# Fedomn/sqlrs

Hardware: AMD Instinct MI355X
Metric: Mrows/sec for filter->hash-join->group-by pipeline; achieved HBM GB/s vs peak (higher is better)
Workload: dtype int64 keys / f64 sum; 1 GPU; C5 filter(val>0.5) -> hash-join(fact x dim on int64 key) -> group-by(key) COUNT,SUM(f64); fact_rows=1000000000, dim_rows=10000000, groups=10000000, parallelism=single GPU

## Files before the change

sqlrs_amd/csrc/agg_partition.hip:

```cpp
#include <algorithm>
#include <cstdlib>
#include <cstring>

#include "agg_partition.hpp"
#include "device_utils.hpp"
#include "radix_part.hpp"

namespace sq {

#ifndef PART_WG_N
#define PART_WG_N 512
#endif
constexpr int PART_WG = PART_WG_N;
#ifndef DENSE_WG_N
#define DENSE_WG_N 1024
#endif
constexpr int DENSE_WG = DENSE_WG_N;
#ifndef HOT_MIN_PEERS_N
#define HOT_MIN_PEERS_N 8
#endif
constexpr int HOT_MIN_PEERS = HOT_MIN_PEERS_N;
constexpr uint64_t LDS_EMPTY = ~0ull;

__device__ __forceinline__ uint32_t bucket_of(uint64_t h, uint32_t P) {
// ... 1351 lines not shown
  out->may_dup = false;
  uint32_t nsplit = 0, nchunk_tables = 0;
  for (uint32_t bkt = 0; bkt < P; bkt++) {
    uint32_t lo = hb[bkt], hi = pr.bucket_end(bkt);
    if (dense && lo == hi) continue;
    if (hi - lo <= split_above) {
      work.insert(work.end(), {bkt, lo, hi, 0xffffffffu});
    } else if (dense) {
      chunk_lo.push_back(nchunk_tables);
      const uint32_t pieces = (uint32_t)ceil_div((int64_t)(hi - lo), (int64_t)chunk);
      for (uint32_t q = 0; q < pieces; q++) {
        const uint32_t c0 = lo + (uint32_t)((uint64_t)(hi - lo) * q / pieces), c1 = lo + (uint32_t)((uint64_t)(hi - lo) * (q + 1) / pieces);
        work.insert(work.end(), {bkt, c0, c1, nchunk_tables++});
      }
      split_bucket.push_back(bkt);
      nsplit++;
    } else {
      for (uint32_t c0 = lo; c0 < hi; c0 += chunk) work.insert(work.end(), {bkt, c0, std::min(hi, c0 + chunk), nsplit});
      split_bucket.push_back(bkt);
      nsplit++;
    }
  }
  chunk_lo.push_back(nchunk_tables);
  if (nsplit) {
    std::vector<uint32_t> ord(work.size() / 4), sorted(work.size());
    for (uint32_t i = 0; i < ord.size(); i++) ord[i] = i;
    std::stable_sort(ord.begin(), ord.end(), [&](uint32_t a, uint32_t b) {
      return work[4 * a + 2] - work[4 * a + 1] > work[4 * b + 2] - work[4 * b + 1];
    });
    for (size_t i = 0; i < ord.size(); i++) std::memcpy(&sorted[4 * i], &work[4 * ord[i]], 16);
    work.swap(sorted);
  }
  const uint32_t nwork = (uint32_t)(work.size() / 4);
  BufP dwork = ctx->alloc(4 * work.size() + 16);
  SQ_HIP(hipMemcpyAsync(dwork->p, work.data(), 4 * work.size(), hipMemcpyHostToDevice, ctx->stream));
  const uint32_t nslots_h = dense ? cap : cap + 2;
  SplitTables stb;
  BufP stb_key, stb_first, stb_acc, dsplit;
  BufP dchunk_lo;
  if (nsplit && dense) {
    const int64_t total = (int64_t)nchunk_tables * nslots_h;
    stb_first = ctx->alloc(4 * (size_t)total);
    stb_acc = ctx->alloc(8 * (size_t)total * (size_t)std::max(spec.n_acc, 1));
    stb.first = stb_first->as<unsigned int>();
    stb.acc = stb_acc->as<unsigned long long>();
    stb.nsplit = nchunk_tables;
    dsplit = ctx->alloc(4 * (size_t)nsplit);
    dchunk_lo = ctx->alloc(4 * ((size_t)nsplit + 1));
    SQ_HIP(hipMemcpyAsync(dsplit->p, split_bucket.data(), 4 * (size_t)nsplit, hipMemcpyHostToDevice, ctx->stream));
    SQ_HIP(hipMemcpyAsync(dchunk_lo->p, chunk_lo.data(), 4 * ((size_t)nsplit + 1), hipMemcpyHostToDevice, ctx->stream));
  } else if (nsplit) {
    const int64_t total = (int64_t)nsplit * nslots_h;
    stb_key = ctx->alloc(8 * (size_t)total);
    stb_first = ctx->alloc(4 * (size_t)total);
    stb_acc = ctx->alloc(8 * (size_t)total * (size_t)std::max(spec.n_acc, 1));
    stb.key = stb_key->as<unsigned long long>();
    stb.first = stb_first->as<unsigned int>();
    stb.acc = stb_acc->as<unsigned long long>();
    stb.nsplit = nsplit;
    split_init_kernel<<<dim3((unsigned)ceil_div(total, 256)), dim3(256), 0, ctx->stream>>>(stb, total, spec.n_acc, prm);
    SQ_HIP(hipGetLastError());
  }
  out->gkey = ctx->alloc(8 * (size_t)gcap);
  out->gfirst = ctx->alloc(4 * (size_t)gcap);
  out->gvalid = in.key_validity ? ctx->alloc((size_t)gcap) : nullptr;
  out->gacc = ctx->alloc(8 * (size_t)gcap * (size_t)std::max(spec.n_acc, 1));
  out->gcap = gcap;
  if (!out->ov_rows) out->ov_rows = ctx->alloc(4 * (size_t)std::max<int64_t>(n, 1));
  ctx->agg_route[pr.pack.kbits ? Ctx::AR_PACKED : Ctx::AR_UNPACKED]++;
  ctx->agg_route[Ctx::AR_FLAGS] += pf != nullptr;
  ctx->agg_route[Ctx::AR_REC] += pr.rec != nullptr;
  ctx->agg_route[Ctx::AR_IN_PLACE] += in_place;
  ctx->agg_route[Ctx::AR_JOIN] += join_mode;
  ctx->agg_route[Ctx::AR_JOIN_MULT] += prm.partner_mult != nullptr;
  ctx->agg_route[Ctx::AR_SPLIT] += nsplit > 0;
  {
    ProfScope ps(ctx, "lds_agg");
#define SQ_LA(NV, FL, JN, NA, C0, C1, PK)                                                                        \
  do {                                                                                                         \
    auto kfn = lds_agg_kernel<NV, FL, JN, NA, C0, C1, PK>;                                                      \
    constexpr bool can_rec = NV == 1 && PK && !FL;                                                             \
    if (can_rec && pr.rec) kfn = lds_agg_kernel<NV, FL, JN, NA, C0, C1, PK, can_rec>;                          \
    else if (pr.rec) fail(SQLRS_ERR_INTERNAL, "record-form partition in a column-form bucket pass");           \
    allow_big_lds(ctx, kfn);                                                                                   \
    kfn<<<dim3(nwork), dim3(PART_WG), lds, ctx->stream>>>(                                                     \
        prm, pr.rec ? pr.rec->as<uint64_t>() : pk->as<uint64_t>(), pi ? pi->as<uint32_t>() : nullptr, pv0 ? pv0->as<uint64_t>() : nullptr,       \
        pv1 ? pv1->as<uint64_t>() : nullptr, pf ? pf->as<uint8_t>() : nullptr, dwork->as<uint32_t>(), P, n,    \
        ctr->as<unsigned long long>(), out->gkey->as<uint64_t>(), out->gfirst->as<uint32_t>(),                 \
        out->gvalid ? out->gvalid->as<uint8_t>() : nullptr, out->gacc->as<uint64_t>(), gcap,                   \
        ctr->as<unsigned long long>() + 1, out->ov_rows->as<uint32_t>(),                                       \
        bp ? bp->key->as<uint64_t>() : nullptr, (bp && bp->flags) ? bp->flags->as<uint8_t>() : nullptr,        \
        bp ? bp->bstart->as<uint32_t>() : nullptr, pr.pack, stb);                                              \
    ctx->agg_route[NA < 0 ? Ctx::AR_PROBE_GENERIC : Ctx::AR_PROBE_SPEC]++;                                     \
    launched = true;                                                                                           \
  } while (0)
#define SQ_LA_J(NV, FL, NA, C0, C1)                                                                            \
  do {                                                                                                         \
    if (pr.pack.kbits) {                                                                                       \
      if (join_mode) SQ_LA(NV, FL, true, NA, C0, C1, true);                                                    \
      else SQ_LA(NV, FL, false, NA, C0, C1, true);                                                             \
    } else {                                                                                                   \
      if (join_mode) SQ_LA(NV, FL, true, NA, C0, C1, false);                                                   \
      else SQ_LA(NV, FL, false, NA, C0, C1, false);                                                            \
    }                                                                                                          \
  } while (0)
    const int nvu = pv1 ? 2 : ((pv0 || pr.rec) ? 1 : 0);
    bool launched = false;
    if (dense && pr.slim.on) {
// ... 131 lines not shown
```

sqlrs_amd/csrc/common.hpp:

```cpp
#pragma once

#include <hip/hip_runtime.h>

#include <cstdint>
#include <cstdlib>
#include <cstring>
#include <map>
#include <set>
#include <memory>
#include <string>
#include <vector>

#include "sqlrs_hip.h"

namespace sq {

inline bool hooks_enabled() {
  static const bool on = [] {
    const char *e = std::getenv("SQLRS_HOOKS");
    return e && e[0] == '1';
  }();
  return on;
}
inline const char *hook(const char *name) { return hooks_enabled() ? std::getenv(name) : nullptr; }
// ... 64 lines not shown
  Buf &operator=(const Buf &) = delete;
  template <class T> T *as() const { return (T *)p; }
};
using BufP = std::shared_ptr<Buf>;
inline BufP buf_view(const BufP &parent, const void *p, size_t bytes) {
  BufP v = std::make_shared<Buf>(parent->ctx, const_cast<void *>(p), bytes);
  v->owned = false;
  v->parent = parent;
  return v;
}

struct ProfEntry {
  const char *name;
  double total_ms = 0;
  int64_t launches = 0;
};
struct ProfPending {
  int entry;
  hipEvent_t a, b;
};

struct Ctx {
  int device = 0;
  hipStream_t stream = nullptr;
  std::string last_error;
  std::shared_ptr<Pool> pool_ref = std::make_shared<Pool>();
  Pool &pool = *pool_ref;
  int num_cus = 256;
  bool prof_on = false;
  std::vector<ProfEntry> prof;
  std::vector<ProfPending> prof_pending;
  std::vector<hipEvent_t> event_pool;
  hipEvent_t order_event = nullptr;
  void *pinned = nullptr;
  size_t pinned_bytes = 0;

  BufP alloc(size_t bytes);
  BufP alloc_zero(size_t bytes);
  BufP zero_block;
  size_t zero_used = 0;
  std::set<const void *> big_lds_set;
  std::map<const void *, int> occ_cache;
  int64_t lb_timeouts = 0;
  int64_t order_lb_fallbacks = 0;
  int lb_backoff = 0;
  int64_t async_conj_batches = 0;
  int64_t async_fast_batches = 0;
  enum AggRoute {
    AR_DENSE, AR_SLIM_RUNS, AR_SLIM_BLK, AR_PROBE_SPEC, AR_PROBE_GENERIC,
    AR_INTERPRETED,
    AR_PACKED, AR_UNPACKED,
    AR_FLAGS,
    AR_REC,
    AR_IN_PLACE,
    AR_JOIN,
    AR_JOIN_MULT,
    AR_SPLIT,
    AR_OVERFLOW_ROWS,
    AR_MERGE_GROUPS,
    AR_PENDING,
    AR_WIDE_PARTS,
    AR_COUNT_
  };
  int64_t agg_route[AR_COUNT_] = {};
  std::shared_ptr<void> small_ring;
  void sync() { SQ_HIP(hipStreamSynchronize(stream)); }
  const void *fetch(const void *dptr, size_t bytes);
  template <class T> T fetch_value(const T *dptr) { return *(const T *)fetch(dptr, sizeof(T)); }
  void *pinned_early = nullptr;
  hipEvent_t early_event = nullptr;
  bool fetch_early(const void *dptr, size_t bytes);
  const void *fetch_early_wait();
  int prof_entry(const char *name);
  void prof_resolve();
};

template <class K> inline void allow_big_lds(Ctx *ctx, K kfn, int bytes = 150 * 1024) {
  const void *f = (const void *)kfn;
  if (ctx->big_lds_set.count(f)) return;
  SQ_HIP(hipFuncSetAttribute(f, hipFuncAttributeMaxDynamicSharedMemorySize, bytes));
  ctx->big_lds_set.insert(f);
}

struct ProfScope {
  Ctx *ctx;
  int entry = -1;
  hipEvent_t a = nullptr, b = nullptr;
  ProfScope(Ctx *c, const char *name);
  ~ProfScope();
};

struct DCol {
  int32_t dtype = SQLRS_NULLTYPE;
  int64_t length = 0;
  int64_t null_count = 0;
  int stride = 1;
  const void *values = nullptr;
  const uint64_t *validity = nullptr;
  const int32_t *offsets = nullptr;
  int64_t data_bytes = 0;
  uint64_t scalar_bits = 0;
  bool scalar_null = false;
  BufP own_values, own_validity, own_offsets;
  bool has_nulls() const { return validity != nullptr && null_count != 0; }
  template <class T> const T *v() const { return (const T *)values; }
};

struct DBatch {
  int64_t rows = 0;
  std::vector<DCol> cols;
};

struct InBatch {
  Ctx *ctx;
  const sqlrs_batch_t *abi;
  std::vector<DCol> cache;
  std::vector<uint8_t> loaded;
  bool host_upload = false;
  const DBatch *shared = nullptr;
  InBatch(Ctx *c, const sqlrs_batch_t *b);
  ~InBatch();
  InBatch(const InBatch &) = delete;
// ... 65 lines not shown
```

sqlrs_amd/csrc/ctx.hip:

```cpp
#include <cstdlib>

#include <array>
#include <atomic>
#include <mutex>
#include <unordered_set>

#include "common.hpp"
#include "host_stage.hpp"
#include "prims.hpp"
#include "small_async.hpp"

extern "C" void sqlrs_batch_release(sqlrs_batch_t *batch);
namespace sq {

static size_t pool_size_class(size_t bytes) {
  if (bytes < 512) return 512;
  if (bytes <= (1u << 20)) {
    size_t s = 512;
    while (s < bytes) s <<= 1;
    return s;
  }
  return round_up(bytes, (size_t)2 << 20);
}

// ... 153 lines not shown
const void *Ctx::fetch(const void *dptr, size_t bytes) {
  if (bytes > pinned_bytes) fail(SQLRS_ERR_INTERNAL, "fetch too large");
  SQ_HIP(hipMemcpyAsync(pinned, dptr, bytes, hipMemcpyDeviceToHost, stream));
  sync();
  return pinned;
}
bool Ctx::fetch_early(const void *dptr, size_t bytes) {
  if (bytes > pinned_bytes) return false;
  if (!pinned_early && hipHostMalloc(&pinned_early, pinned_bytes, hipHostMallocDefault) != hipSuccess) {
    pinned_early = nullptr;
    return false;
  }
  if (!early_event && hipEventCreateWithFlags(&early_event, hipEventDisableTiming) != hipSuccess) {
    early_event = nullptr;
    return false;
  }
  SQ_HIP(hipMemcpyAsync(pinned_early, dptr, bytes, hipMemcpyDeviceToHost, stream));
  SQ_HIP(hipEventRecord(early_event, stream));
  return true;
}
const void *Ctx::fetch_early_wait() {
  SQ_HIP(hipEventSynchronize(early_event));
  return pinned_early;
}
int Ctx::prof_entry(const char *name) {
  for (size_t i = 0; i < prof.size(); i++)
    if (prof[i].name == name || std::strcmp(prof[i].name, name) == 0) return (int)i;
  prof.push_back(ProfEntry{name});
  return (int)prof.size() - 1;
}
void Ctx::prof_resolve() {
  if (prof_pending.empty()) return;
  sync();
  for (auto &p : prof_pending) {
    float ms = 0;
    if (hipEventElapsedTime(&ms, p.a, p.b) == hipSuccess) {
      prof[p.entry].total_ms += ms;
      prof[p.entry].launches++;
    }
    event_pool.push_back(p.a);
    event_pool.push_back(p.b);
  }
  prof_pending.clear();
}

ProfScope::ProfScope(Ctx *c, const char *name) : ctx(c) {
  if (!c->prof_on) return;
  entry = c->prof_entry(name);
  auto get = [&]() {
    if (!c->event_pool.empty()) {
      hipEvent_t e = c->event_pool.back();
      c->event_pool.pop_back();
      return e;
    }
    hipEvent_t e;
    SQ_HIP(hipEventCreate(&e));
    return e;
  };
  a = get();
  b = get();
  (void)hipEventRecord(a, c->stream);
}
ProfScope::~ProfScope() {
  if (entry < 0) return;
  (void)hipEventRecord(b, ctx->stream);
  ctx->prof_pending.push_back(ProfPending{entry, a, b});
  if (ctx->prof_pending.size() > 4096) {
    try {
      ctx->prof_resolve();
    } catch (...) {
    }
  }
}

Expr expr_from_abi(const sqlrs_expr_t *e) {
  Expr x;
  if (!e || e->num_nodes <= 0 || !e->nodes) fail(SQLRS_ERR_INTERNAL, "empty expression");
  x.nodes.assign(e->nodes, e->nodes + e->num_nodes);
  x.strings.resize(x.nodes.size());
  for (size_t i = 0; i < x.nodes.size(); i++) {
    if (x.nodes[i].s) x.strings[i] = x.nodes[i].s;
    x.nodes[i].s = nullptr;
  }
  return x;
}

static void copy_in(Ctx *ctx, void *dst, const void *src, size_t bytes, int mem) {
  if (!bytes) return;
  SQ_HIP(hipMemcpyAsync(dst, src, bytes,
                        mem == SQLRS_MEM_HOST ? hipMemcpyHostToDevice : hipMemcpyDeviceToDevice,
                        ctx->stream));
}

DCol upload_column(Ctx *ctx, const sqlrs_column_t &c, bool force_copy) {
  DCol d;
  d.dtype = c.dtype;
  d.length = c.length;
  d.null_count = c.validity ? c.null_count : 0;
// ... 501 lines not shown
  int n = 0;
  if (hipGetDeviceCount(&n) != hipSuccess || n <= 0 || device_id < 0 || device_id >= n)
    return SQLRS_ERR_DEVICE;
  hipDeviceProp_t prop;
  if (hipGetDeviceProperties(&prop, device_id) != hipSuccess) return SQLRS_ERR_DEVICE;
  if (std::string(prop.gcnArchName).rfind("gfx950", 0) != 0) return SQLRS_ERR_DEVICE;
  if (hipSetDevice(device_id) != hipSuccess) return SQLRS_ERR_DEVICE;
  auto *c = new sqlrs_ctx();
  c->device = device_id;
  c->pool.device = device_id;
  c->num_cus = prop.multiProcessorCount;
  if (hipStreamCreateWithFlags(&c->stream, hipStreamNonBlocking) != hipSuccess ||
      hipHostMalloc(&c->pinned, 65536, hipHostMallocDefault) != hipSuccess) {
    delete c;
    return SQLRS_ERR_DEVICE;
  }
  c->pinned_bytes = 65536;
  if (const char *e = std::getenv("SQLRS_POOL_RESERVE_GB")) {
    const size_t bytes = (size_t)(std::atof(e) * (double)(1ull << 30));
    void *p = nullptr;
    if (bytes && hipMalloc(&p, bytes) == hipSuccess) {
      c->pool.arena = (uint8_t *)p;
      c->pool.arena_bytes = bytes;
    }
  }
  *out = c;
  return SQLRS_OK;
}

void sqlrs_ctx_destroy(sqlrs_ctx_t *ctx) {
  if (!ctx) return;
  (void)hipSetDevice(ctx->device);
  (void)hipStreamSynchronize(ctx->stream);
  for (auto &p : ctx->prof_pending) {
    (void)hipEventDestroy(p.a);
    (void)hipEventDestroy(p.b);
  }
  for (auto e : ctx->event_pool) (void)hipEventDestroy(e);
  if (ctx->order_event) (void)hipEventDestroy(ctx->order_event);
  ctx->zero_block.reset();
  ctx->pool.trim();
  if (ctx->pool.arena && ctx->pool.live_bytes == 0) {
    ctx->pool.free_blocks.clear();
    (void)hipFree(ctx->pool.arena);
    ctx->pool.arena = nullptr;
  }
  ctx->pool.closed = true;
  if (ctx->pinned) (void)hipHostFree(ctx->pinned);
  if (ctx->pinned_early) (void)hipHostFree(ctx->pinned_early);
  if (ctx->early_event) (void)hipEventDestroy(ctx->early_event);
  (void)hipStreamDestroy(ctx->stream);
  delete ctx;
}

const char *sqlrs_last_error(const sqlrs_ctx_t *ctx) { return ctx ? ctx->last_error.c_str() : ""; }

int sqlrs_ctx_synchronize(sqlrs_ctx_t *ctx) {
  return guard(ctx, [&] {
    ctx->sync();
    sa_drain(ctx);
  });
}
void *sqlrs_ctx_stream(sqlrs_ctx_t *ctx) { return (void *)ctx->stream; }

static int order_streams(sqlrs_ctx_t *ctx, hipStream_t first, hipStream_t then) {
  return guard(ctx, [&] {
    SQ_HIP(hipSetDevice(ctx->device));
    if (!ctx->order_event) SQ_HIP(hipEventCreateWithFlags(&ctx->order_event, hipEventDisableTiming));
    SQ_HIP(hipEventRecord(ctx->order_event, first));
    SQ_HIP(hipStreamWaitEvent(then, ctx->order_event, 0));
  });
}
int sqlrs_ctx_wait_stream(sqlrs_ctx_t *ctx, void *producer_stream) {
  return order_streams(ctx, (hipStream_t)producer_stream, ctx->stream);
}
int sqlrs_ctx_release_to_stream(sqlrs_ctx_t *ctx, void *consumer_stream) {
  return order_streams(ctx, ctx->stream, (hipStream_t)consumer_stream);
}
int64_t sqlrs_ctx_pool_bytes(const sqlrs_ctx_t *ctx) {
  return (int64_t)(ctx->pool.live_bytes + ctx->pool.cached_bytes);
}
void sqlrs_ctx_pool_trim(sqlrs_ctx_t *ctx) {
  (void)hipStreamSynchronize(ctx->stream);
// ... 381 lines not shown
```

sqlrs_amd/csrc/gather.hip:

```cpp
#include "common.hpp"
#include "device_utils.hpp"
#include "prims.hpp"

namespace sq {

template <class T, class I>
__global__ __launch_bounds__(BLOCK) void gather_kernel(const T *__restrict__ src,
                                                       const uint64_t *__restrict__ src_validity,
                                                       const I *__restrict__ idx,
                                                       const uint64_t *__restrict__ idx_validity,
                                                       int64_t n, T *__restrict__ out,
                                                       uint64_t *__restrict__ out_validity) {
  int64_t i = blockIdx.x * (int64_t)blockDim.x + threadIdx.x;
  bool in_range = i < n;
  bool valid = in_range;
  I s = 0;
  if (in_range) {
    if (idx_validity) valid = (idx_validity[i >> 6] >> (i & 63)) & 1;
    if (valid) {
      s = idx[i];
      if (src_validity) valid = (src_validity[s >> 6] >> (s & 63)) & 1;
    }
    out[i] = valid ? src[s] : T(0);
  }
// ... 180 lines not shown
  if (K > 2) {
    u64x2 b;
    b.x = c2[i];
    b.y = K > 3 ? c3[i] : 0ull;
    *(u64x2 *)(rows + (size_t)W * i + 2) = b;
  }
}
template <int K>
__global__ __launch_bounds__(BLOCK) void gather_rows_kernel(const uint64_t *__restrict__ rows, const uint32_t *__restrict__ idx,
                                                            int64_t n, uint64_t *__restrict__ o0, uint64_t *__restrict__ o1,
                                                            uint64_t *__restrict__ o2, uint64_t *__restrict__ o3) {
  constexpr int W = K <= 2 ? 2 : 4, U = 4;
  const int64_t base = blockIdx.x * (int64_t)(BLOCK * U) + threadIdx.x;
  uint32_t s[U];
#pragma unroll
  for (int u = 0; u < U; u++) s[u] = __builtin_nontemporal_load(idx + min(base + u * BLOCK, n - 1));
  u64x2 a[U], b[U];
#pragma unroll
  for (int u = 0; u < U; u++) {
    a[u] = *(const u64x2 *)(rows + (size_t)W * s[u]);
    if (K > 2) b[u] = *(const u64x2 *)(rows + (size_t)W * s[u] + 2);
  }
#pragma unroll
  for (int u = 0; u < U; u++) {
    const int64_t i = base + u * BLOCK;
    if (i >= n) continue;
    o0[i] = a[u].x;
    o1[i] = a[u].y;
    if (K > 2) o2[i] = b[u].x;
    if (K > 3) o3[i] = b[u].y;
  }
}

bool gather_columns_packed(Ctx *ctx, std::vector<DCol> &cols, int64_t src_rows, const uint32_t *idx, int64_t n) {
  const int k = (int)cols.size();
  if (k < 2 || k > 4 || n < (1 << 18)) return false;
  for (const DCol &c : cols)
    if (width_of(c.dtype) != 8 || c.stride == 0 || (c.validity && c.null_count != 0) || c.length != src_rows) return false;
  const int w = k <= 2 ? 2 : 4;
  BufP rows = ctx->alloc(8 * (size_t)w * (size_t)src_rows);
  const uint64_t *p[4] = {nullptr, nullptr, nullptr, nullptr};
  for (int i = 0; i < k; i++) p[i] = cols[(size_t)i].v<uint64_t>();
  dim3 b(BLOCK), gp((unsigned)ceil_div(src_rows, BLOCK)), gg((unsigned)ceil_div(n, BLOCK * 4));
  std::vector<DCol> outs((size_t)k);
  uint64_t *o[4] = {nullptr, nullptr, nullptr, nullptr};
  for (int i = 0; i < k; i++) {
    DCol &d = outs[(size_t)i];
    d.dtype = cols[(size_t)i].dtype;
    d.length = n;
    d.null_count = 0;
    d.own_values = ctx->alloc(8 * (size_t)n + 16);
    d.values = d.own_values->p;
    o[i] = d.own_values->as<uint64_t>();
  }
  uint64_t *r = rows->as<uint64_t>();
  switch (k) {
  case 2:
    pack_rows_kernel<2><<<gp, b, 0, ctx->stream>>>(p[0], p[1], p[2], p[3], src_rows, r);
    gather_rows_kernel<2><<<gg, b, 0, ctx->stream>>>(r, idx, n, o[0], o[1], o[2], o[3]);
    break;
  case 3:
    pack_rows_kernel<3><<<gp, b, 0, ctx->stream>>>(p[0], p[1], p[2], p[3], src_rows, r);
    gather_rows_kernel<3><<<gg, b, 0, ctx->stream>>>(r, idx, n, o[0], o[1], o[2], o[3]);
    break;
  default:
    pack_rows_kernel<4><<<gp, b, 0, ctx->stream>>>(p[0], p[1], p[2], p[3], src_rows, r);
    gather_rows_kernel<4><<<gg, b, 0, ctx->stream>>>(r, idx, n, o[0], o[1], o[2], o[3]);
  }
  SQ_HIP(hipGetLastError());
  cols = std::move(outs);
  return true;
}

__global__ void count_clear_kernel(const uint64_t *__restrict__ bits, int64_t rows, int64_t nwords,
                                   unsigned long long *out) {
  int64_t i = blockIdx.x * (int64_t)blockDim.x + threadIdx.x;
  uint64_t c = 0;
  for (int64_t w = i; w < nwords; w += (int64_t)gridDim.x * blockDim.x) {
    uint64_t v = ~bits[w];
    int64_t rem = rows - w * 64;
    if (rem < 64) v &= (1ull << rem) - 1;
    c += (uint64_t)__popcll(v);
  }
  c = wave_sum_u64(c);
  if (lane_id() == 0 && c) atomicAdd(out, (unsigned long long)c);
}
int64_t count_clear_bits(Ctx *ctx, const uint64_t *bits, int64_t rows) {
  if (!bits || rows == 0) return 0;
  BufP out = ctx->alloc_zero(8);
  int64_t nwords = ceil_div(rows, 64);
  unsigned blocks = (unsigned)std::min<int64_t>(ceil_div(nwords, 256), 2048);
  count_clear_kernel<<<dim3(blocks), dim3(256), 0, ctx->stream>>>(
      bits, rows, nwords, out->as<unsigned long long>());
  SQ_HIP(hipGetLastError());
  return (int64_t)ctx->fetch_value(out->as<uint64_t>());
}

__global__ void append_bits_kernel(const uint64_t *__restrict__ src, int64_t n, int64_t dst_off,
                                   unsigned long long *__restrict__ dst, int all_ones) {
  int64_t i = blockIdx.x * (int64_t)blockDim.x + threadIdx.x;
  int64_t nw = (n + 63) >> 6;
  if (i >= nw) return;
  uint64_t v = all_ones ? ~0ull : src[i];
// ... 200 lines not shown
```

sqlrs_amd/csrc/hashagg_op.hip:

```cpp
#include <cstdlib>

#include "agg_partition.hpp"
#include "agg_state.hpp"
#include "common.hpp"
#include "device_utils.hpp"
#include "host_stage.hpp"
#include "prims.hpp"

using namespace sq;

namespace {

struct AggSpec {
  int func = 0, distinct = 0;
  int32_t return_dtype = 0;
  Expr arg;
  GrowBuf acc, nn;
  bool track_nn = false;
  int32_t acc_dtype = 0;
  int argcol = -1;
  struct StrBatch {
    DCol col;
    BufP gid;
    int64_t n;
// ... 253 lines not shown
    int col = pg.col_of_agg[i];
    int cc = pg.cnt_of_col[(size_t)col];
    if (s.func == SQLRS_AGG_COUNT) {
      s.nn.ensure(ctx, G, 0);
      agg_update_count(ctx, s.nn, rg, nullptr, (const int64_t *)cell(cc), g);
      continue;
    }
    if (pg.col_nullable[(size_t)col]) start_tracking(ctx, s, G, nnew);
    if (s.track_nn) {
      s.nn.ensure(ctx, G, 0);
      agg_update_count(ctx, s.nn, rg, nullptr, (const int64_t *)cell(cc), g);
    }
    int ac = pg.acc_of_agg[i];
    if (s.func == SQLRS_AGG_SUM) {
      s.acc_dtype = s.return_dtype;
      s.acc.ensure(ctx, G, 0);
      agg_update_sum(ctx, s.acc, s.acc_dtype, rg, cell(ac), nullptr, g);
    } else {
      s.acc_dtype = pg.col_dtype[(size_t)col];
      s.acc.ensure(ctx, G, acc_identity(s));
      agg_update_minmax(ctx, s.acc, SQLRS_UINT64 , s.func == SQLRS_AGG_MIN, rg,
                        cell(ac), nullptr, g);
    }
  }
}

static void flush_pending(sqlrs_hash_agg *a) {
  if (!a->pending.active) return;
  PendingGroups pg = std::move(a->pending);
  a->pending = PendingGroups();
  merge_groups(a, pg);
}

static DBatch emit_pending(sqlrs_hash_agg *a) {
  Ctx *ctx = a->ctx;
  PendingGroups &pg = a->pending;
  PartAggOutput &po = pg.po;
  int64_t G = po.groups;
  DBatch o;
  o.rows = G;
  for (const DCol &k : pg.keyvals) o.cols.push_back(k);
  auto cell = [&](int acc) { return po.gacc->as<uint64_t>() + (size_t)acc * (size_t)po.gcap; };
  for (size_t i = 0; i < a->aggs.size(); i++) {
    AggSpec &s = a->aggs[i];
    int col = pg.col_of_agg[i];
    int cc = pg.cnt_of_col[(size_t)col];
    if (s.func == SQLRS_AGG_COUNT) {
      o.cols.push_back(agg_finalize_raw(ctx, s.func, SQLRS_INT64, cell(cc), nullptr, G, po.gacc));
      continue;
    }
    const uint64_t *nn = pg.col_nullable[(size_t)col] ? cell(cc) : nullptr;
    int32_t dt = s.func == SQLRS_AGG_SUM ? s.return_dtype : pg.col_dtype[(size_t)col];
    DCol c = agg_finalize_raw(ctx, s.func, dt, cell(pg.acc_of_agg[i]), nn, G, po.gacc);
    c.dtype = s.return_dtype;
    o.cols.push_back(c);
  }
  if (G > 1 && !a->any_order) {
    ProfScope ps(ctx, "agg_order_groups");
    BufP perm = ctx->alloc(4 * (size_t)G);
    int bits = 1;
    while (bits < 32 && (1ull << bits) <= (uint64_t)std::max<int64_t>(a->rows_seen, 1)) bits++;
    radix_sort_index_u32(ctx, po.gfirst->as<uint32_t>(), G, bits, perm->as<uint32_t>());
    if (!gather_columns_packed(ctx, o.cols, G, perm->as<uint32_t>(), G))
      for (DCol &c : o.cols) c = gather_column(ctx, c, perm->p, false, nullptr, G);
  }
  return o;
}

static DCol distinct_column(sqlrs_hash_agg *a, sqlrs_hash_agg::DistinctAgg &d, int64_t G) {
  Ctx *ctx = a->ctx;
  sqlrs_batch_t *dd = nullptr, *res = nullptr;
  int st = sqlrs_hash_agg_finish(d.dedup, SQLRS_MEM_DEVICE, &dd);
  if (st != SQLRS_OK) fail(st, ctx->last_error);
  const int nk = (int)a->group_by.size();
  std::vector<sqlrs_expr_node_t> nodes((size_t)nk + 1);
  std::vector<sqlrs_expr_t> gb((size_t)nk);
  std::memset(nodes.data(), 0, sizeof(sqlrs_expr_node_t) * nodes.size());
  for (int i = 0; i < nk; i++) {
    nodes[(size_t)i].op = SQLRS_EXPR_INPUT_REF;
    nodes[(size_t)i].index = i;
    gb[(size_t)i].nodes = &nodes[(size_t)i];
    gb[(size_t)i].num_nodes = 1;
    gb[(size_t)i].reserved = 0;
  }
  sqlrs_agg_func_t af;
  std::memset(&af, 0, sizeof(af));
  if (d.func == SQLRS_AGG_COUNT) {
    nodes[(size_t)nk].op = SQLRS_EXPR_CONSTANT;
    nodes[(size_t)nk].dtype = SQLRS_INT64;
    nodes[(size_t)nk].i = 1;
    af.func = SQLRS_AGG_COUNT;
    af.return_dtype = SQLRS_INT64;
  } else {
    nodes[(size_t)nk].op = SQLRS_EXPR_INPUT_REF;
    nodes[(size_t)nk].index = nk;
    af.func = SQLRS_AGG_SUM;
    af.return_dtype = d.return_dtype;
// ... 627 lines not shown
    flush_pending(a);
    int64_t G = a->st.ngroups;
    DBatch o;
    o.rows = G;
    for (size_t c = 0; c < a->key_parts.size(); c++) {
      if (a->key_parts[c].empty()) {
        DCol e = make_null_column(ctx, a->key_dtypes[c], 0);
        e.null_count = 0;
        o.cols.push_back(e);
        continue;
      }
      std::vector<const DCol *> parts;
      for (const DCol &p : a->key_parts[c]) parts.push_back(&p);
      o.cols.push_back(concat_columns(ctx, parts));
    }
    for (AggSpec &s : a->aggs) {
      if (s.func == SQLRS_AGG_COUNT) {
        s.nn.ensure(ctx, std::max<int64_t>(G, 1), 0);
        o.cols.push_back(agg_finalize_values(ctx, s.func, SQLRS_INT64, s.nn, nullptr, G));
        continue;
      }
      if (!s.strs.empty() || s.return_dtype == SQLRS_UTF8) {
        o.cols.push_back(finalize_utf8_minmax(ctx, s, G));
        continue;
      }
      int32_t dt = s.acc_dtype ? s.acc_dtype : s.return_dtype;
      s.acc.ensure(ctx, std::max<int64_t>(G, 1), acc_identity(s));
      DCol c = agg_finalize_values(ctx, s.func, dt, s.acc, s.track_nn ? &s.nn : nullptr, G);
      c.dtype = s.return_dtype;
      o.cols.push_back(c);
    }
    if (!a->in_order && G > 1 && !a->any_order) {
      ProfScope ps(ctx, "agg_order_groups");
      agg_refresh_gfirst(ctx, a->st);
      BufP keys = ctx->alloc(8 * (size_t)G), perm = ctx->alloc(4 * (size_t)G);
      SQ_HIP(hipMemcpyAsync(keys->p, a->st.gfirst.buf->p, 8 * (size_t)G, hipMemcpyDeviceToDevice, ctx->stream));
      iota_u32(ctx, perm->as<uint32_t>(), G);
      int bits = 1;
      while (bits < 64 && (1ull << bits) <= (uint64_t)std::max<int64_t>(a->rows_seen, 1)) bits++;
      radix_sort_pairs(ctx, keys->as<uint64_t>(), perm->as<uint32_t>(), G, 0, bits, true);
      if (!gather_columns_packed(ctx, o.cols, G, perm->as<uint32_t>(), G))
        for (DCol &c : o.cols) c = gather_column(ctx, c, perm->p, false, nullptr, G);
    }
    place_aggregate_columns(a, o);
    return o;
  }
}

int sqlrs_hash_agg_set_group_order(sqlrs_hash_agg_t *a, int group_order) {
  return guard(a->ctx, [&] {
    if (group_order != SQLRS_GROUP_ORDER_FIRST_SEEN && group_order != SQLRS_GROUP_ORDER_ANY)
      fail(SQLRS_ERR_INTERNAL, "unknown group order");
    if (!a->distinct_aggs.empty() && group_order == SQLRS_GROUP_ORDER_ANY)
      fail(SQLRS_ERR_INTERNAL, "DISTINCT aggregates line up by first-seen order: SQLRS_GROUP_ORDER_ANY not supported");
    a->any_order = group_order == SQLRS_GROUP_ORDER_ANY;
  });
}

int sqlrs_hash_agg_set_filter(sqlrs_hash_agg_t *a, const sqlrs_expr_t *filter) {
  return guard(a->ctx, [&] {
    if (a->saw_batch || !a->staged.empty() || a->hstage.has_schema)
      fail(SQLRS_ERR_INTERNAL, "set_filter after the first batch");
    a->has_filter = filter && filter->num_nodes > 0;
    if (a->has_filter) a->filter = expr_from_abi(filter);
    for (sqlrs_hash_agg *p : a->parts) {
      int st = sqlrs_hash_agg_set_filter(p, filter);
      if (st != SQLRS_OK) fail(st, a->ctx->last_error);
    }
  });
}
int64_t sqlrs_hash_agg_filter_fused_batches(const sqlrs_hash_agg_t *a) {
  return a->parts.empty() ? a->filter_fused_batches : a->parts[0]->filter_fused_batches;
}

void sqlrs_hash_agg_destroy(sqlrs_hash_agg_t *a) { delete a; }
// ... 417 lines not shown
```

sqlrs_amd/csrc/prims.hpp:

```cpp
#pragma once

#include <functional>

#include "common.hpp"

namespace sq {

void exclusive_scan_u32(Ctx *ctx, const uint32_t *in, int64_t n, uint64_t *out64, uint32_t *out32,
                        uint64_t *total);

struct Selection {
  int64_t rows = 0;
  int64_t count = 0;
  const uint64_t *bits = nullptr;
  BufP own_bits;
  BufP tile_off;
};
Selection selection_from_mask(Ctx *ctx, const DCol &mask);
Selection selection_from_clear_bits(Ctx *ctx, const uint64_t *bits, int64_t rows);
Selection selection_from_set_bits(Ctx *ctx, const uint64_t *bits, int64_t rows);
void selection_finish(Ctx *ctx, Selection &s);
DCol compact_column(Ctx *ctx, const DCol &c, const Selection &s);
BufP selection_indices_u32(Ctx *ctx, const Selection &s);
BufP selection_indices_u64(Ctx *ctx, const Selection &s);

bool filter_fast_path(Ctx *ctx, const Expr &e, const std::function<const DCol &(int)> &col,
                      int64_t rows, int *col_index, Selection *sel, DCol *out_col);

DCol gather_column(Ctx *ctx, const DCol &src, const void *idx, bool idx_is_u64,
                   const uint64_t *idx_validity, int64_t n);
bool gather_columns_packed(Ctx *ctx, std::vector<DCol> &cols, int64_t src_rows, const uint32_t *idx, int64_t n);
DCol concat_columns(Ctx *ctx, const std::vector<const DCol *> &parts);
DCol copy_column(Ctx *ctx, const DCol &c);
void sort_perm_by_utf8(Ctx *ctx, const DCol &c, const uint64_t *valid, int desc, uint32_t *perm, uint64_t *keys,
                       int64_t n);
DCol materialize_scalar(Ctx *ctx, const DCol &c, int64_t rows);
int64_t count_clear_bits(Ctx *ctx, const uint64_t *bits, int64_t rows);

DCol eval_expr(Ctx *ctx, const Expr &e, const std::function<const DCol &(int)> &col, int64_t rows,
               bool materialize);

struct NKeys {
  int64_t rows = 0;
  BufP keys;
  const uint64_t *validity = nullptr;
  BufP own_validity;
  bool exact = true;
  int32_t dtype = SQLRS_INT64;
};
NKeys normalize_keys(Ctx *ctx, const std::vector<DCol> &cols, int64_t rows);
NKeys normalize_keys_strong(Ctx *ctx, const std::vector<DCol> &cols, int64_t rows);

void radix_sort_pairs(Ctx *ctx, uint64_t *keys, uint32_t *vals, int64_t n, int begin_bit,
                      int end_bit, bool keys_below_end_bit = false);
void radix_sort_index_u32(Ctx *ctx, const uint32_t *keys, int64_t n, int bits, uint32_t *perm);
void iota_u32(Ctx *ctx, uint32_t *out, int64_t n);
bool order_fast(Ctx *ctx, const DCol &key, int desc, const DCol *carry, int64_t n, DCol *key_out, DCol *carry_out,
                BufP *perm, bool want_perm, bool *in_order = nullptr);
bool order_composite(Ctx *ctx, const std::vector<const DCol *> &keys, const std::vector<int> &desc, const DCol *carry, int64_t n,
                     std::vector<DCol> *keys_out, DCol *carry_out, BufP *perm, bool want_perm, bool *in_order);

}
```

sqlrs_amd/csrc/radix_part.hip:

```cpp
#include <cstdio>
#include <cstdlib>

#include "device_utils.hpp"
#include "radix_part.hpp"
#include "radix_part_kernels.hpp"

namespace sq {

namespace {

struct Level {
  std::vector<int64_t> seg_mat, seg_start;
  std::vector<uint32_t> seg_tiles, seg_tile_base;
  int64_t mat_entries = 0;
  uint32_t num_tiles = 0, nseg = 0;
  std::vector<uint8_t> blob;
  BufP dev, tiles;
  const int64_t *d_seg_start = nullptr, *d_seg_mat = nullptr;
  const uint32_t *d_seg_tiles = nullptr, *d_seg_tile_base = nullptr;
};

Level plan_level(const std::vector<int64_t> &seg_start, uint32_t digits, int RP_TILE) {
  Level L;
  L.seg_start = seg_start;
// ... 474 lines not shown
          so.chunk_len, so.chunk_dig, so.counter, so.max_chunks, so.max_chunks, digits2, (uint32_t)CAP, (uint32_t)RP_TILE,
          L2.d_seg_tiles, L2.d_seg_tile_base, plan->as<ChunkPlan>(), (Tile *)L2.tiles->p, tile_chunk->as<uint32_t>());
      SQ_HIP(hipGetLastError());
      const uint64_t *ht = (const uint64_t *)ctx->fetch(totals->p, 24);
      const uint64_t ntiles = ht[0], kept = ht[1], overflow = ht[2];
      if (overflow) return false;
      L2.num_tiles = (uint32_t)ntiles;
      L2.mat_entries = (int64_t)ntiles * digits2;
      out->n = (int64_t)kept;
      out->P = P;
      if (kept == 0) {
        out->bstart_host.assign((size_t)P + 1, 0u);
        out->bstart = nullptr;
        return true;
      }
      const size_t np = (size_t)kept + 1024;
      PartitionedRows::Slim &sl = out->slim;
      sl = PartitionedRows::Slim();
      sl.rows = slim_alloc(np, sl.buf0, sl.buf1);
      SlimLaunch sln;
      sln.in.rows = so.rows;
      sln.in.tile_chunk = tile_chunk->as<uint32_t>();
      sln.in.cstart = so.cstart;
      sln.out.rows = sl.rows;
      sln.kshift = so.kshift;
      sln.rbits = kp.rbits;
      BufP offs2;
      BufP premat = ctx->alloc(4 * (size_t)L2.mat_entries);
      rp_hist_from_chunks_kernel<<<dim3((unsigned)ceil_div(L2.mat_entries, 256)), dim3(256), 0, ctx->stream>>>(
          so.hist, tile_chunk->as<uint32_t>(), L2.mat_entries, digits2, premat->as<uint32_t>());
      SQ_HIP(hipGetLastError());
      EarlyStarts es;
      early_starts_for(L2, digits2, (int64_t)kept, es);
      exec_level(2, digits2, L2, RpIn(), RpOut(), (int64_t)kept, &offs2, premat, &sln, &es.queue);
      sl.nzstart = ctx->alloc(4 * (size_t)L2.mat_entries);
      sl.nzbt = ctx->alloc(4 * (size_t)L2.mat_entries);
      sl.nzcount = ctx->alloc(4 * (size_t)P);
      sl.bcol = ctx->alloc(4 * (size_t)P);
      ProfScope ps_runs(ctx, "rp_slim_runs");
      rp_slim_runs_kernel<<<dim3(P), dim3(256), 0, ctx->stream>>>(
          offs2->as<uint32_t>(), L2.mat_entries, sln.total->as<uint64_t>(), L2.d_seg_mat, L2.d_seg_tiles, L2.d_seg_tile_base,
          tile_chunk->as<uint32_t>(), so.chunk_base, digits2, sl.nzstart->as<uint32_t>(), sl.nzbt->as<uint32_t>(),
          sl.nzcount->as<uint32_t>(), sl.bcol->as<uint32_t>());
      SQ_HIP(hipGetLastError());
      if (hook("SQLRS_RP_TRACE"))
        std::fprintf(stderr, "[rp_slim] keys %p vals %p chunks %p %p rows %p %p kept %llu tiles %u\n", (const void *)in.keys, in.vals[0],
                     cb0 ? cb0->p : nullptr, cb1 ? cb1->p : nullptr, sl.buf0 ? sl.buf0->p : nullptr, sl.buf1 ? sl.buf1->p : nullptr,
                     (unsigned long long)kept, L2.num_tiles);
      sl.tile = (uint32_t)RP_TILE;
      sl.on = true;
      out->key = out->v0 = out->v1 = out->idx = out->flags = out->rec = nullptr;
      out->bstart = finish_starts(es, L2, offs2, digits2, (int64_t)kept, &out->bstart_host);
      return true;
    }
    if (chunked) {
      const size_t pool_rows = (size_t)max_chunks * (CAP + RP_CHUNK_SKEW) + (size_t)1024 * cwgs;
      BufP ck = staggered(8 * pool_rows, 0), c0 = nv >= 1 ? staggered(8 * pool_rows, 1) : nullptr,
           c1 = nv >= 2 ? staggered(8 * pool_rows, 2) : nullptr, ci = pack ? nullptr : staggered(4 * pool_rows, 3);
      BufP clen = ctx->alloc_zero(4 * (size_t)max_chunks);
      BufP cdig = ctx->alloc(4 * (size_t)max_chunks);
      BufP ctr = ctx->alloc_zero(8);
      ChunkOut co;
      co.arena = (uint32_t)arena;
      co.key = ck->as<uint64_t>();
      co.v0 = c0 ? c0->as<uint64_t>() : nullptr;
      co.v1 = c1 ? c1->as<uint64_t>() : nullptr;
      co.idx = ci ? ci->as<uint32_t>() : nullptr;
      co.chunk_len = clen->as<uint32_t>();
      co.chunk_dig = cdig->as<uint32_t>();
      co.counter = ctr->as<unsigned int>();
      co.base_chunks = (uint32_t)max_chunks;
      co.max_chunks = (uint32_t)max_chunks;
      co.cap = (uint32_t)CAP;
      const int psrc = !in.filter.col ? -1 : ((nv >= 1 && (const void *)in.filter.col == in.vals[0]) ? 1 : 3);
      const char *h2_e = hook("SQLRS_RP_H2");
      const bool h2_unpacked = !pack && nv == 1 && psrc != 3 &&
                               (size_t)RP_TILE * (8 * 2 + 4 + 2) + (size_t)WG * (4 + 4 + 8 + 8) + (size_t)WG * 8 + (size_t)P * 4 <= 159 * 1024;
// ... 152 lines not shown
```

sqlrs_amd/csrc/radix_part.hpp:

```cpp
#pragma once

#include "common.hpp"
#include "prims.hpp"

namespace sq {

struct KeyPack {
  uint64_t kmin = 0, kmask = 0;
  uint32_t kbits = 0;
  uint32_t dense = 0, rbits = 0;
  uint64_t range = 0;
  unsigned int *oob = nullptr;
  unsigned long long *ov_count = nullptr;
  uint32_t *ov_rows = nullptr;
  uint32_t ov_cap = 0;
};
#if defined(__HIPCC__)
__device__ __forceinline__ void key_out_of_range(const KeyPack &kp, uint32_t row) {
  if (!kp.ov_rows) {
    *kp.oob = 1u;
    return;
  }
  const unsigned long long peers = __ballot(1);
  const int leader = __builtin_ctzll(peers);
// ... 53 lines not shown
bool fusable_row_filter(const Expr &e, InBatch &ib, RowFilter *rf);

struct PartitionInput {
  const uint64_t *keys = nullptr;
  const uint64_t *key_validity = nullptr;
  int64_t n = 0;
  int nv = 0;
  const void *vals[2] = {nullptr, nullptr};
  const uint64_t *val_validity[2] = {nullptr, nullptr};
  bool build_side = false;
  KeyPack pack;
  RowFilter filter;
};

struct PartitionedRows {
  int64_t n = 0;
  uint32_t P = 0;
  BufP key, v0, v1, idx, flags;
  BufP rec;
  BufP bstart;
  std::vector<uint32_t> bstart_host;
  std::vector<uint32_t> bend_host;
  uint32_t bucket_end(uint32_t b) const { return bend_host.empty() ? bstart_host[b + 1] : bend_host[b]; }
  KeyPack pack;
  struct Slim {
    bool on = false;
    BufP buf0, buf1;
    SlimRowsView rows;
    BufP nzstart, nzbt;
    BufP nzcount, bcol;
    uint32_t tile = 0;
    BufP blk_bt;
    uint32_t log_b = 0;
  } slim;
};

bool partition_rows(Ctx *ctx, const PartitionInput &in, uint32_t P_wanted, PartitionedRows *out);

}
```

Baseline: 99030 Mrows/s.

## Overlap slim-runs, work uploads and row packing on a side stream

Adds a side stream with fork/join events. The slim-runs kernel in radix partitioning, the host-to-device uploads of the work list for the LDS aggregation, and the pack_rows kernel used for group reordering are queued there so they can run concurrently with the scatter and sort on the main stream. It also preallocates an upload area so the uploads avoid allocator calls on the critical path. This adds stream and event management, and if synchronisation is missed there is a risk of races or buffer-lifetime issues.

```diff
diff --git a/sqlrs_amd/csrc/agg_partition.hip b/sqlrs_amd/csrc/agg_partition.hip
--- a/sqlrs_amd/csrc/agg_partition.hip
+++ b/sqlrs_amd/csrc/agg_partition.hip
@@ -1407,8 +1407,21 @@
     work.swap(sorted);
   }
   const uint32_t nwork = (uint32_t)(work.size() / 4);
-  BufP dwork = ctx->alloc(4 * work.size() + 16);
-  SQ_HIP(hipMemcpyAsync(dwork->p, work.data(), 4 * work.size(), hipMemcpyHostToDevice, ctx->stream));
+  SideWork *side = (pr.slim.side && pr.slim.side->on()) ? pr.slim.side.get() : nullptr;
+  size_t room_used = 0;
+  if (side) {
+    const size_t need = round_up(4 * work.size() + 16, 256) + (nsplit ? round_up(4 * (size_t)nsplit, 256) + round_up(4 * ((size_t)nsplit + 1), 256) : 0);
+    if (!pr.slim.side_room || need > pr.slim.side_room->cap) side = nullptr;
+  }
+  const hipStream_t up = side ? side->stream() : ctx->stream;
+  auto upload_room = [&](size_t bytes) -> BufP {
+    if (!side) return ctx->alloc(bytes);
+    BufP v = buf_view(pr.slim.side_room, pr.slim.side_room->as<uint8_t>() + room_used, bytes);
+    room_used += round_up(bytes, 256);
+    return v;
+  };
+  BufP dwork = upload_room(4 * work.size() + 16);
+  SQ_HIP(hipMemcpyAsync(dwork->p, work.data(), 4 * work.size(), hipMemcpyHostToDevice, up));
   const uint32_t nslots_h = dense ? cap : cap + 2;
   SplitTables stb;
   BufP stb_key, stb_first, stb_acc, dsplit;
@@ -1420,10 +1433,10 @@
     stb.first = stb_first->as<unsigned int>();
     stb.acc = stb_acc->as<unsigned long long>();
     stb.nsplit = nchunk_tables;
-    dsplit = ctx->alloc(4 * (size_t)nsplit);
-    dchunk_lo = ctx->alloc(4 * ((size_t)nsplit + 1));
-    SQ_HIP(hipMemcpyAsync(dsplit->p, split_bucket.data(), 4 * (size_t)nsplit, hipMemcpyHostToDevice, ctx->stream));
-    SQ_HIP(hipMemcpyAsync(dchunk_lo->p, chunk_lo.data(), 4 * ((size_t)nsplit + 1), hipMemcpyHostToDevice, ctx->stream));
+    dsplit = upload_room(4 * (size_t)nsplit);
+    dchunk_lo = upload_room(4 * ((size_t)nsplit + 1));
+    SQ_HIP(hipMemcpyAsync(dsplit->p, split_bucket.data(), 4 * (size_t)nsplit, hipMemcpyHostToDevice, up));
+    SQ_HIP(hipMemcpyAsync(dchunk_lo->p, chunk_lo.data(), 4 * ((size_t)nsplit + 1), hipMemcpyHostToDevice, up));
   } else if (nsplit) {
     const int64_t total = (int64_t)nsplit * nslots_h;
     stb_key = ctx->alloc(8 * (size_t)total);
@@ -1449,6 +1462,7 @@
   ctx->agg_route[Ctx::AR_JOIN] += join_mode;
   ctx->agg_route[Ctx::AR_JOIN_MULT] += prm.partner_mult != nullptr;
   ctx->agg_route[Ctx::AR_SPLIT] += nsplit > 0;
+  if (pr.slim.side) pr.slim.side->join();
   {
     ProfScope ps(ctx, "lds_agg");
 #define SQ_LA(NV, FL, JN, NA, C0, C1, PK)                                                                        \
diff --git a/sqlrs_amd/csrc/common.hpp b/sqlrs_amd/csrc/common.hpp
--- a/sqlrs_amd/csrc/common.hpp
+++ b/sqlrs_amd/csrc/common.hpp
@@ -120,6 +120,9 @@
   std::vector<ProfPending> prof_pending;
   std::vector<hipEvent_t> event_pool;
   hipEvent_t order_event = nullptr;
+  hipStream_t side_stream = nullptr;
+  hipEvent_t side_fork = nullptr, side_join = nullptr;
+  hipStream_t side();
   void *pinned = nullptr;
   size_t pinned_bytes = 0;
 
@@ -174,8 +177,30 @@
   Ctx *ctx;
   int entry = -1;
   hipEvent_t a = nullptr, b = nullptr;
-  ProfScope(Ctx *c, const char *name);
+  hipStream_t stream = nullptr;
+  ProfScope(Ctx *c, const char *name, hipStream_t on = nullptr);
   ~ProfScope();
+};
+
+inline bool side_stream_enabled() {
+  const char *e = hook("SQLRS_SIDE_STREAM");
+  return !(e && e[0] == '0');
+}
+
+struct SideWork {
+  Ctx *ctx;
+  bool open = false;
+  std::vector<BufP> held;
+  explicit SideWork(Ctx *c, bool use = true);
+  ~SideWork();
+  SideWork(const SideWork &) = delete;
+  SideWork &operator=(const SideWork &) = delete;
+  bool on() const { return open; }
+  hipStream_t stream() const { return open ? ctx->side_stream : ctx->stream; }
+  void hold(const BufP &b) {
+    if (b) held.push_back(b);
+  }
+  void join();
 };
 
 struct DCol {
diff --git a/sqlrs_amd/csrc/ctx.hip b/sqlrs_amd/csrc/ctx.hip
--- a/sqlrs_amd/csrc/ctx.hip
+++ b/sqlrs_amd/csrc/ctx.hip
@@ -209,6 +209,7 @@
 void Ctx::prof_resolve() {
   if (prof_pending.empty()) return;
   sync();
+  if (side_stream) SQ_HIP(hipStreamSynchronize(side_stream));
   for (auto &p : prof_pending) {
     float ms = 0;
     if (hipEventElapsedTime(&ms, p.a, p.b) == hipSuccess) {
@@ -221,7 +222,46 @@
   prof_pending.clear();
 }
 
-ProfScope::ProfScope(Ctx *c, const char *name) : ctx(c) {
+hipStream_t Ctx::side() {
+  if (!side_stream) {
+    hipStream_t s = nullptr;
+    hipEvent_t f = nullptr, j = nullptr;
+    if (hipStreamCreateWithFlags(&s, hipStreamNonBlocking) != hipSuccess ||
+        hipEventCreateWithFlags(&f, hipEventDisableTiming) != hipSuccess ||
+        hipEventCreateWithFlags(&j, hipEventDisableTiming) != hipSuccess) {
+      if (j) (void)hipEventDestroy(j);
+      if (f) (void)hipEventDestroy(f);
+      if (s) (void)hipStreamDestroy(s);
+      fail(SQLRS_ERR_DEVICE, "side stream: stream or event creation failed");
+    }
+    side_stream = s;
+    side_fork = f;
+    side_join = j;
+  }
+  return side_stream;
+}
+
+SideWork::SideWork(Ctx *c, bool use) : ctx(c) {
+  if (!use || !side_stream_enabled()) return;
+  hipStream_t s = c->side();
+  SQ_HIP(hipEventRecord(c->side_fork, c->stream));
+  SQ_HIP(hipStreamWaitEvent(s, c->side_fork, 0));
+  open = true;
+}
+void SideWork::join() {
+  if (open) {
+    open = false;
+    if (hipEventRecord(ctx->side_join, ctx->side_stream) != hipSuccess ||
+        hipStreamWaitEvent(ctx->stream, ctx->side_join, 0) != hipSuccess) {
+      (void)hipGetLastError();
+      (void)hipStreamSynchronize(ctx->side_stream);
+    }
+  }
+  held.clear();
+}
+SideWork::~SideWork() { join(); }
+
+ProfScope::ProfScope(Ctx *c, const char *name, hipStream_t on) : ctx(c), stream(on ? on : c->stream) {
   if (!c->prof_on) return;
   entry = c->prof_entry(name);
   auto get = [&]() {
@@ -236,11 +276,11 @@
   };
   a = get();
   b = get();
-  (void)hipEventRecord(a, c->stream);
+  (void)hipEventRecord(a, stream);
 }
 ProfScope::~ProfScope() {
   if (entry < 0) return;
-  (void)hipEventRecord(b, ctx->stream);
+  (void)hipEventRecord(b, stream);
   ctx->prof_pending.push_back(ProfPending{entry, a, b});
   if (ctx->prof_pending.size() > 4096) {
     try {
@@ -808,6 +848,7 @@
   if (!ctx) return;
   (void)hipSetDevice(ctx->device);
   (void)hipStreamSynchronize(ctx->stream);
+  if (ctx->side_stream) (void)hipStreamSynchronize(ctx->side_stream);
   for (auto &p : ctx->prof_pending) {
     (void)hipEventDestroy(p.a);
     (void)hipEventDestroy(p.b);
@@ -825,6 +866,9 @@
   if (ctx->pinned) (void)hipHostFree(ctx->pinned);
   if (ctx->pinned_early) (void)hipHostFree(ctx->pinned_early);
   if (ctx->early_event) (void)hipEventDestroy(ctx->early_event);
+  if (ctx->side_fork) (void)hipEventDestroy(ctx->side_fork);
+  if (ctx->side_join) (void)hipEventDestroy(ctx->side_join);
+  if (ctx->side_stream) (void)hipStreamDestroy(ctx->side_stream);
   (void)hipStreamDestroy(ctx->stream);
   delete ctx;
 }
diff --git a/sqlrs_amd/csrc/gather.hip b/sqlrs_amd/csrc/gather.hip
--- a/sqlrs_amd/csrc/gather.hip
+++ b/sqlrs_amd/csrc/gather.hip
@@ -236,16 +236,35 @@
   }
 }
 
-bool gather_columns_packed(Ctx *ctx, std::vector<DCol> &cols, int64_t src_rows, const uint32_t *idx, int64_t n) {
+bool pack_rows_shape(const std::vector<DCol> &cols, int64_t src_rows, int64_t n) {
   const int k = (int)cols.size();
   if (k < 2 || k > 4 || n < (1 << 18)) return false;
   for (const DCol &c : cols)
     if (width_of(c.dtype) != 8 || c.stride == 0 || (c.validity && c.null_count != 0) || c.length != src_rows) return false;
+  return true;
+}
+bool pack_rows(Ctx *ctx, const std::vector<DCol> &cols, int64_t src_rows, int64_t n, hipStream_t stream, PackedRows *out) {
+  if (!pack_rows_shape(cols, src_rows, n)) return false;
+  const int k = (int)cols.size();
   const int w = k <= 2 ? 2 : 4;
-  BufP rows = ctx->alloc(8 * (size_t)w * (size_t)src_rows);
+  out->rows = ctx->alloc(8 * (size_t)w * (size_t)src_rows);
+  out->k = k;
+  out->src_rows = src_rows;
   const uint64_t *p[4] = {nullptr, nullptr, nullptr, nullptr};
   for (int i = 0; i < k; i++) p[i] = cols[(size_t)i].v<uint64_t>();
-  dim3 b(BLOCK), gp((unsigned)ceil_div(src_rows, BLOCK)), gg((unsigned)ceil_div(n, BLOCK * 4));
+  dim3 b(BLOCK), gp((unsigned)ceil_div(src_rows, BLOCK));
+  uint64_t *r = out->rows->as<uint64_t>();
+  switch (k) {
+  case 2: pack_rows_kernel<2><<<gp, b, 0, stream>>>(p[0], p[1], p[2], p[3], src_rows, r); break;
+  case 3: pack_rows_kernel<3><<<gp, b, 0, stream>>>(p[0], p[1], p[2], p[3], src_rows, r); break;
+  default: pack_rows_kernel<4><<<gp, b, 0, stream>>>(p[0], p[1], p[2], p[3], src_rows, r);
+  }
+  SQ_HIP(hipGetLastError());
+  return true;
+}
+void gather_packed_rows(Ctx *ctx, const PackedRows &pk, std::vector<DCol> &cols, const uint32_t *idx, int64_t n) {
+  const int k = pk.k;
+  dim3 b(BLOCK), gg((unsigned)ceil_div(n, BLOCK * 4));
   std::vector<DCol> outs((size_t)k);
   uint64_t *o[4] = {nullptr, nullptr, nullptr, nullptr};
   for (int i = 0; i < k; i++) {
@@ -257,22 +276,19 @@
     d.values = d.own_values->p;
     o[i] = d.own_values->as<uint64_t>();
   }
-  uint64_t *r = rows->as<uint64_t>();
+  const uint64_t *r = pk.rows->as<uint64_t>();
   switch (k) {
-  case 2:
-    pack_rows_kernel<2><<<gp, b, 0, ctx->stream>>>(p[0], p[1], p[2], p[3], src_rows, r);
-    gather_rows_kernel<2><<<gg, b, 0, ctx->stream>>>(r, idx, n, o[0], o[1], o[2], o[3]);
-    break;
-  case 3:
-    pack_rows_kernel<3><<<gp, b, 0, ctx->stream>>>(p[0], p[1], p[2], p[3], src_rows, r);
-    gather_rows_kernel<3><<<gg, b, 0, ctx->stream>>>(r, idx, n, o[0], o[1], o[2], o[3]);
-    break;
-  default:
-    pack_rows_kernel<4><<<gp, b, 0, ctx->stream>>>(p[0], p[1], p[2], p[3], src_rows, r);
-    gather_rows_kernel<4><<<gg, b, 0, ctx->stream>>>(r, idx, n, o[0], o[1], o[2], o[3]);
+  case 2: gather_rows_kernel<2><<<gg, b, 0, ctx->stream>>>(r, idx, n, o[0], o[1], o[2], o[3]); break;
+  case 3: gather_rows_kernel<3><<<gg, b, 0, ctx->stream>>>(r, idx, n, o[0], o[1], o[2], o[3]); break;
+  default: gather_rows_kernel<4><<<gg, b, 0, ctx->stream>>>(r, idx, n, o[0], o[1], o[2], o[3]);
   }
   SQ_HIP(hipGetLastError());
   cols = std::move(outs);
+}
+bool gather_columns_packed(Ctx *ctx, std::vector<DCol> &cols, int64_t src_rows, const uint32_t *idx, int64_t n) {
+  PackedRows pk;
+  if (!pack_rows(ctx, cols, src_rows, n, ctx->stream, &pk)) return false;
+  gather_packed_rows(ctx, pk, cols, idx, n);
   return true;
 }
 
diff --git a/sqlrs_amd/csrc/hashagg_op.hip b/sqlrs_amd/csrc/hashagg_op.hip
--- a/sqlrs_amd/csrc/hashagg_op.hip
+++ b/sqlrs_amd/csrc/hashagg_op.hip
@@ -309,6 +309,27 @@
   merge_groups(a, pg);
 }
 
+template <class SortFn>
+static void order_group_columns(Ctx *ctx, std::vector<DCol> &cols, int64_t G, const uint32_t *perm, SortFn &&sort) {
+  const bool shape = pack_rows_shape(cols, G, G);
+  PackedRows pk;
+  bool packed = false;
+  SideWork sw(ctx, shape);
+  if (sw.on()) {
+    ProfScope ps(ctx, "agg_pack_rows", sw.stream());
+    packed = pack_rows(ctx, cols, G, G, sw.stream(), &pk);
+  }
+  sort();
+  sw.join();
+  if (shape && !packed) {
+    ProfScope ps(ctx, "agg_pack_rows");
+    packed = pack_rows(ctx, cols, G, G, ctx->stream, &pk);
+  }
+  if (packed) gather_packed_rows(ctx, pk, cols, perm, G);
+  else
+    for (DCol &c : cols) c = gather_column(ctx, c, perm, false, nullptr, G);
+}
+
 static DBatch emit_pending(sqlrs_hash_agg *a) {
   Ctx *ctx = a->ctx;
   PendingGroups &pg = a->pending;
@@ -337,9 +358,8 @@
     BufP perm = ctx->alloc(4 * (size_t)G);
     int bits = 1;
     while (bits < 32 && (1ull << bits) <= (uint64_t)std::max<int64_t>(a->rows_seen, 1)) bits++;
-    radix_sort_index_u32(ctx, po.gfirst->as<uint32_t>(), G, bits, perm->as<uint32_t>());
-    if (!gather_columns_packed(ctx, o.cols, G, perm->as<uint32_t>(), G))
-      for (DCol &c : o.cols) c = gather_column(ctx, c, perm->p, false, nullptr, G);
+    order_group_columns(ctx, o.cols, G, perm->as<uint32_t>(),
+                        [&] { radix_sort_index_u32(ctx, po.gfirst->as<uint32_t>(), G, bits, perm->as<uint32_t>()); });
   }
   return o;
 }
@@ -1033,15 +1053,16 @@
     }
     if (!a->in_order && G > 1 && !a->any_order) {
       ProfScope ps(ctx, "agg_order_groups");
-      agg_refresh_gfirst(ctx, a->st);
-      BufP keys = ctx->alloc(8 * (size_t)G), perm = ctx->alloc(4 * (size_t)G);
-      SQ_HIP(hipMemcpyAsync(keys->p, a->st.gfirst.buf->p, 8 * (size_t)G, hipMemcpyDeviceToDevice, ctx->stream));
-      iota_u32(ctx, perm->as<uint32_t>(), G);
-      int bits = 1;
-      while (bits < 64 && (1ull << bits) <= (uint64_t)std::max<int64_t>(a->rows_seen, 1)) bits++;
-      radix_sort_pairs(ctx, keys->as<uint64_t>(), perm->as<uint32_t>(), G, 0, bits, true);
-      if (!gather_columns_packed(ctx, o.cols, G, perm->as<uint32_t>(), G))
-        for (DCol &c : o.cols) c = gather_column(ctx, c, perm->p, false, nullptr, G);
+      BufP perm = ctx->alloc(4 * (size_t)G);
+      order_group_columns(ctx, o.cols, G, perm->as<uint32_t>(), [&] {
+        agg_refresh_gfirst(ctx, a->st);
+        BufP keys = ctx->alloc(8 * (size_t)G);
+        SQ_HIP(hipMemcpyAsync(keys->p, a->st.gfirst.buf->p, 8 * (size_t)G, hipMemcpyDeviceToDevice, ctx->stream));
+        iota_u32(ctx, perm->as<uint32_t>(), G);
+        int bits = 1;
+        while (bits < 64 && (1ull << bits) <= (uint64_t)std::max<int64_t>(a->rows_seen, 1)) bits++;
+        radix_sort_pairs(ctx, keys->as<uint64_t>(), perm->as<uint32_t>(), G, 0, bits, true);
+      });
     }
     place_aggregate_columns(a, o);
     return o;
diff --git a/sqlrs_amd/csrc/prims.hpp b/sqlrs_amd/csrc/prims.hpp
--- a/sqlrs_amd/csrc/prims.hpp
+++ b/sqlrs_amd/csrc/prims.hpp
@@ -30,6 +30,14 @@
 DCol gather_column(Ctx *ctx, const DCol &src, const void *idx, bool idx_is_u64,
                    const uint64_t *idx_validity, int64_t n);
 bool gather_columns_packed(Ctx *ctx, std::vector<DCol> &cols, int64_t src_rows, const uint32_t *idx, int64_t n);
+struct PackedRows {
+  BufP rows;
+  int k = 0;
+  int64_t src_rows = 0;
+};
+bool pack_rows_shape(const std::vector<DCol> &cols, int64_t src_rows, int64_t n);
+bool pack_rows(Ctx *ctx, const std::vector<DCol> &cols, int64_t src_rows, int64_t n, hipStream_t stream, PackedRows *out);
+void gather_packed_rows(Ctx *ctx, const PackedRows &pk, std::vector<DCol> &cols, const uint32_t *idx, int64_t n);
 DCol concat_columns(Ctx *ctx, const std::vector<const DCol *> &parts);
 DCol copy_column(Ctx *ctx, const DCol &c);
 void sort_perm_by_utf8(Ctx *ctx, const DCol &c, const uint64_t *valid, int desc, uint32_t *perm, uint64_t *keys,
diff --git a/sqlrs_amd/csrc/radix_part.hip b/sqlrs_amd/csrc/radix_part.hip
--- a/sqlrs_amd/csrc/radix_part.hip
+++ b/sqlrs_amd/csrc/radix_part.hip
@@ -530,17 +530,30 @@
       SQ_HIP(hipGetLastError());
       EarlyStarts es;
       early_starts_for(L2, digits2, (int64_t)kept, es);
-      exec_level(2, digits2, L2, RpIn(), RpOut(), (int64_t)kept, &offs2, premat, &sln, &es.queue);
-      sl.nzstart = ctx->alloc(4 * (size_t)L2.mat_entries);
-      sl.nzbt = ctx->alloc(4 * (size_t)L2.mat_entries);
-      sl.nzcount = ctx->alloc(4 * (size_t)P);
-      sl.bcol = ctx->alloc(4 * (size_t)P);
-      ProfScope ps_runs(ctx, "rp_slim_runs");
-      rp_slim_runs_kernel<<<dim3(P), dim3(256), 0, ctx->stream>>>(
-          offs2->as<uint32_t>(), L2.mat_entries, sln.total->as<uint64_t>(), L2.d_seg_mat, L2.d_seg_tiles, L2.d_seg_tile_base,
-          tile_chunk->as<uint32_t>(), so.chunk_base, digits2, sl.nzstart->as<uint32_t>(), sl.nzbt->as<uint32_t>(),
-          sl.nzcount->as<uint32_t>(), sl.bcol->as<uint32_t>());
-      SQ_HIP(hipGetLastError());
+      auto queue_runs = [&](const BufP &offs, hipStream_t st) {
+        sl.nzstart = ctx->alloc(4 * (size_t)L2.mat_entries);
+        sl.nzbt = ctx->alloc(4 * (size_t)L2.mat_entries);
+        sl.nzcount = ctx->alloc(4 * (size_t)P);
+        sl.bcol = ctx->alloc(4 * (size_t)P);
+        ProfScope ps_runs(ctx, "rp_slim_runs", st);
+        rp_slim_runs_kernel<<<dim3(P), dim3(256), 0, st>>>(
+            offs->as<uint32_t>(), L2.mat_entries, sln.total->as<uint64_t>(), L2.d_seg_mat, L2.d_seg_tiles, L2.d_seg_tile_base,
+            tile_chunk->as<uint32_t>(), so.chunk_base, digits2, sl.nzstart->as<uint32_t>(), sl.nzbt->as<uint32_t>(),
+            sl.nzcount->as<uint32_t>(), sl.bcol->as<uint32_t>());
+        SQ_HIP(hipGetLastError());
+      };
+      const bool side_on = side_stream_enabled();
+      const std::function<void(const BufP &)> before_scatter = [&](const BufP &offs) {
+        if (side_on) {
+          sl.side = std::make_shared<SideWork>(ctx);
+          queue_runs(offs, sl.side->stream());
+          sl.side_room = ctx->alloc(16 * ((size_t)P + (size_t)kept / 16384 + 2) + 8 * ((size_t)P + 1) + 4 * 256);
+          for (const BufP &b : {offs, sln.total, L2.dev, tile_chunk, cbase}) sl.side->hold(b);
+        }
+        es.queue(offs);
+      };
+      exec_level(2, digits2, L2, RpIn(), RpOut(), (int64_t)kept, &offs2, premat, &sln, &before_scatter);
+      if (!side_on) queue_runs(offs2, ctx->stream);
       if (hook("SQLRS_RP_TRACE"))
         std::fprintf(stderr, "[rp_slim] keys %p vals %p chunks %p %p rows %p %p kept %llu tiles %u\n", (const void *)in.keys, in.vals[0],
                      cb0 ? cb0->p : nullptr, cb1 ? cb1->p : nullptr, sl.buf0 ? sl.buf0->p : nullptr, sl.buf1 ? sl.buf1->p : nullptr,
diff --git a/sqlrs_amd/csrc/radix_part.hpp b/sqlrs_amd/csrc/radix_part.hpp
--- a/sqlrs_amd/csrc/radix_part.hpp
+++ b/sqlrs_amd/csrc/radix_part.hpp
@@ -109,6 +109,8 @@
     uint32_t tile = 0;
     BufP blk_bt;
     uint32_t log_b = 0;
+    std::shared_ptr<SideWork> side;
+    BufP side_room;
   } slim;
 };
 
```

Result: no change. 98490 Mrows/s, median of 2 (-0.5%).
